# bxlab/bx-python

Measured on AMD Instinct MI355X. Metric: M overlap-queries/s at 100M x 10M intervals (count-only), higher is better.
Workload: dtype int32

## Files before the change

bx-python_amd/bxmi/_ffi.py:

```python
import ctypes as C
import os

import numpy as np

_HERE = os.path.dirname(os.path.abspath(__file__))
LIB_PATH = os.environ.get("BXMI_LIB") or os.path.join(_HERE, "libbxmi.so")

OK, EINVAL, ENOMEM, EHIP, ESTATE, ERANGE = 0, 1, 2, 3, 4, 5


class BxmiError(RuntimeError):
    def __init__(self, code, msg):
        super().__init__("libbxmi error %d: %s" % (code, msg))
        self.code = code


vp = C.c_void_p
i32, i64 = C.c_int32, C.c_int64
_p = C.POINTER

_SIGNATURES = {
    "bxmi_device_count": [_p(C.c_int)],
    "bxmi_set_device": [C.c_int],
    "bxmi_get_device": [_p(C.c_int)],
# ... 14 lines not shown
    "bxmi_ivl_append_dev": [vp, vp, vp, i64, vp],
    "bxmi_ivl_seal": [vp, vp],
    "bxmi_ivl_size": [vp, _p(i64)],
    "bxmi_ivl_has_reversed": [vp, _p(C.c_int)],
    "bxmi_ivl_order": [vp, vp],
    "bxmi_ivl_order_dev": [vp, _p(vp), _p(vp), _p(vp)],
    "bxmi_ivl_count": [vp, vp, vp, i64, vp, _p(i64)],
    "bxmi_ivl_count_dev": [vp, vp, vp, i64, vp, vp, vp],
    "bxmi_ivl_count_multi_dev": [vp, C.c_int, vp, vp, vp, vp, vp, vp],
    "bxmi_ivl_slice_state": [vp, _p(C.c_int), vp],
    "bxmi_ivl_dense_state": [vp, _p(C.c_int), vp],
    "bxmi_ivl_flat_state": [vp, _p(C.c_int), _p(i64)],
    "bxmi_ivl_sparse_state": [vp, _p(C.c_int), _p(i64), _p(C.c_int)],
    "bxmi_ivl_count_width": [vp, _p(C.c_int), _p(i64)],
    "bxmi_ivl_order_state": [vp, _p(C.c_int), _p(i64)],
    "bxmi_ivl_find": [vp, vp, vp, i64, vp, vp, i64, _p(i64)],
    "bxmi_ivl_find_dev": [vp, vp, vp, i64, vp, vp, i64, _p(i64), vp],
    "bxmi_ivl_find_one": [vp, i32, i32, vp, i64, _p(i64)],
    "bxmi_ivl_neighbors": [vp, i32, i32, C.c_int, vp, i64, _p(i64)],
    "bxmi_ivl_neighbors_batch": [vp, vp, i64, i32, i32, C.c_int, vp, vp, vp],
    "bxmi_ivl_neighbors_batch_dev": [vp, vp, i64, i32, i32, C.c_int, vp, vp, vp, vp],
    "bxmi_ivl_clusters": [vp, vp, i32, _p(i64), vp, vp, vp, vp],
    "bxmi_chainmap_create": [_p(vp), i64, vp, vp, vp, vp, vp, vp, vp, vp, vp],
    "bxmi_chainmap_destroy": [vp],
    "bxmi_chainmap_info": [vp, _p(i64), _p(i64), _p(i64)],
    "bxmi_chainmap_map": [vp, vp, vp, i64, i32, C.c_int, C.c_double, vp, vp, vp, vp, vp, i64, _p(i64)],
    "bxmi_chainmap_map_dev": [vp, vp, vp, i64, i32, C.c_int, C.c_double, vp, vp, vp, vp, vp, i64, _p(i64), vp],
    "bxmi_scores_create": [i64, _p(vp)],
    "bxmi_scores_destroy": [vp],
    "bxmi_scores_info": [vp, _p(i64)],
# ... 237 lines not shown
```

bx-python_amd/bxmi/intervals.py:

```python
import ctypes as C

import numpy as np

from . import _ffi
from ._ffi import as_i32, call, ptr


class IntervalIndex:

    def __init__(self):
        _ffi.require_gpu()
        h = C.c_void_p()
        call("bxmi_ivl_create", C.byref(h))
        self._h = h
        self._n = 0
        self._sealed = False
        self._one_buf = np.empty(4096, dtype=np.int32)

    def close(self):
        if getattr(self, "_h", None):
            _ffi.load().bxmi_ivl_destroy(self._h)
            self._h = None

    def __del__(self):
# ... 51 lines not shown
        st, hc, k = C.c_int(0), C.c_int64(0), C.c_int(0)
        call("bxmi_ivl_sparse_state", self._h, C.byref(st), C.byref(hc), C.byref(k))
        return st.value, hc.value, k.value

    def count_width(self):
        self._ready()
        bits, wide = C.c_int(0), C.c_int64(0)
        call("bxmi_ivl_count_width", self._h, C.byref(bits), C.byref(wide))
        return bits.value, wide.value

    def order_state(self):
        self._ready()
        sk, seen = C.c_int(0), C.c_int64(0)
        call("bxmi_ivl_order_state", self._h, C.byref(sk), C.byref(seen))
        return sk.value, seen.value

    def dense_state(self):
        self._ready()
        st, worst = C.c_int(0), (C.c_int64 * 2)()
        call("bxmi_ivl_dense_state", self._h, C.byref(st), worst)
        return st.value, list(worst)

    def order(self):
        self._ready()
        out = np.empty(self._n, dtype=np.int32)
        if self._n:
            call("bxmi_ivl_order", self._h, ptr(out))
        return out

    def count(self, qs, qe, want_counts=True):
# ... 129 lines not shown
```

bx-python_amd/csrc/count_dense.hpp:

```cpp
#pragma once
#include "offset_cells.hpp"

namespace bxmi {

constexpr int BD_UNIT_LOG2 = 19;
constexpr int BD_RSHIFT = 19;
constexpr int BD_MARGIN = 8192;
constexpr int BD_MAX_F = 6;
constexpr int BD_MAX_SHIFT = 19;
constexpr int BD_OV_MAX = 32704;
constexpr int BD_TABLE_FROM_FIRST = 2, BD_TABLE_FROM_LAST = 6;
constexpr int BD_THREADS = 1024;
constexpr int BD_LONG_SLOTS = 64;
constexpr int BD_LONG_CAP = 320;
constexpr int BD_HDR_QS = 6;

struct BdLayout {
    int nce, ncs;
    int bitsE, bitsS, metaE, metaS, hdr, ov, bytes;
    int ov_cap;
};

__host__ __device__ inline BdLayout bd_layout(int unit_log2)
{
// ... 1131 lines not shown
        for (int j = 0; j < 4; j++) b[j] = c[j] < 0xFFu ? c[j] : 0xFFu;
        reinterpret_cast<unsigned *>(out)[idx4] = b[0] | (b[1] << 8) | (b[2] << 16) | (b[3] << 24);
    } else {
        bd_v2u o;
        o.x = c[0] | (c[1] << 16), o.y = c[2] | (c[3] << 16);
        reinterpret_cast<bd_v2u *>(out)[idx4] = o;
    }
}

template <bool W8, int DEPTH, bool WIDE = false, int THREADS = BD_THREADS, bool TOT = false>
__global__ __launch_bounds__(THREADS) void bw_search_kernel(const BmSeg *__restrict__ segs, const int4 *__restrict__ items,
                                                               const int *__restrict__ n_items, const unsigned short *__restrict__ unitT, int64_t ntp,
                                                               const unsigned *__restrict__ recs ,
                                                               unsigned short *__restrict__ out , int tile_log2,
                                                               const unsigned *__restrict__ gate, unsigned *__restrict__ xcd_next ,
                                                               unsigned long long *__restrict__ total_slots = nullptr )
{
    if (gate && *gate == 0) return;
    extern __shared__ __attribute__((aligned(16))) int32_t dyn[];
    __shared__ long long s_red[TOT ? THREADS / 64 : 1];
    unsigned long long acc = 0ull;
    int acc_seg = -1;
    constexpr int LONG_CAP = THREADS == BD_THREADS ? BD_LONG_CAP : BD_LONG_CAP / 2;
    constexpr int PF = THREADS == BD_THREADS ? BW_PF : 10;
    __shared__ uint2 s_long[LONG_CAP];
    __shared__ int s_nlong, s_next, s_item_next;
    __shared__ __attribute__((aligned(8))) unsigned s_mask[THREADS / 64][BW_MASK_WORDS];
    const int nit = *n_items;
    const int per_xcd = (nit + 7) >> 3;
    const int xcd = (int)(blockIdx.x & 7);
    const int it_lo = xcd * per_xcd, it_hi = it_lo + per_xcd < nit ? it_lo + per_xcd : nit;
    const int lane = lane_id(), wave = __builtin_amdgcn_readfirstlane((int)(threadIdx.x >> 6));
    unsigned *const wmask = s_mask[wave];
    wmask[lane] = 0u, wmask[64 + lane] = 0u;
    if (threadIdx.x == 0) s_item_next = it_lo + (int)atomicAdd(&xcd_next[xcd], 1u);
    __syncthreads();
    int it = __builtin_amdgcn_readfirstlane(s_item_next);
    __syncthreads();
    const unsigned tile_slots = ((1u << tile_log2) + (unsigned)BM_PAD_ROOM) >> 2;
    while (it < it_hi) {
        const int4 item = items[it];
        const int unit = item.x & 0xffff, t0 = item.y, t1 = item.z;
        const BmSeg &sg = segs[item.x >> 16];
        if (TOT && (item.x >> 16) != acc_seg) {
            if (acc_seg >= 0) {
                block_accumulate_i64((long long)acc, s_red, total_slots + (int64_t)acc_seg * PT_SLOTS + (blockIdx.x & (PT_SLOTS - 1)));
                __syncthreads();
            }
            acc = 0ull, acc_seg = item.x >> 16;
        }
        const BmGeom g = sg.g;
        const int cell_log2 = WIDE ? 5 + g.dshift : 5;
        const BpLayout LP = bp_layout(g.shift + g.f, cell_log2, WIDE ? g.stride : 0);
        const unsigned short *__restrict__ runs0 = unitT + (int64_t)unit * ntp;
        const unsigned short *__restrict__ runs1 = runs0 + ntp;
        int B = BW_B;
// ... 397 lines not shown
                    } else {
#pragma unroll
                        for (int j = 0; j < 4; j++)
                            if (k0 + j >= lo && k0 + j < hi) as_global(sg.counts)[k0 + j] = (int)c[j];
                    }
                }
                acc += (long long)c[0] + c[1] + c[2] + c[3];
            }
        }
        __syncthreads();
        it = it_nx;
    }
    if (total_slots && acc_seg >= 0) block_accumulate_i64(acc, red, total_slots + (int64_t)acc_seg * PT_SLOTS + (blockIdx.x & (PT_SLOTS - 1)));
}

template <int THREADS, int ITEMS, bool PAD, bool W8>
__device__ __forceinline__ void bd_unpermute_tile(const unsigned short *__restrict__ cnt ,
                                                  const unsigned short *__restrict__ slots, const BmSeg *__restrict__ segs,
                                                  const unsigned short *__restrict__ tile_seg,
                                                  unsigned long long *__restrict__ total_slots ,
                                                  const unsigned *__restrict__ gate, const unsigned *__restrict__ tend,
                                                  unsigned long long *__restrict__ fb_dev ,
                                                  unsigned long long *__restrict__ fb_host )
{
    constexpr int TILE = THREADS * ITEMS;
    constexpr int STRIDE = PAD ? TILE + BM_PAD_ROOM : TILE;
    static_assert(ITEMS % 8 == 0, "whole 16-byte vectors of 16-bit counts per thread");
    extern __shared__ __attribute__((aligned(16))) int32_t dyn[];
    if (gate && *gate == 0) return;
    unsigned short *vals = reinterpret_cast<unsigned short *>(dyn);
    __shared__ long long red[THREADS / 64];
    const int64_t tile = blockIdx.x;
    const int seg_id = tile_seg[tile];
    const BmSeg &sg = segs[seg_id];
    const int64_t ltile = tile - sg.tile0;
    if (ltile >= sg.ntiles) return;
    unsigned long long *const acc_to = total_slots ? total_slots + (int64_t)seg_id * PT_SLOTS + (blockIdx.x & (PT_SLOTS - 1)) : nullptr;
    const IndexDev ix = sg.ix;
    const BmGeom g = sg.g;
    const int32_t *__restrict__ e_sorted = sg.e_sorted;
    const int32_t BX_GLOBAL *__restrict__ qs_arr = as_global(sg.qs) + ltile * TILE, *__restrict__ qe_arr = as_global(sg.qe) + ltile * TILE;
    int32_t BX_GLOBAL *__restrict__ out = as_global(sg.counts) + ltile * TILE;
    static_assert(!W8 || PAD, "8-bit counts come with the padded layout");
    const unsigned char *vals8 = reinterpret_cast<const unsigned char *>(dyn);
// ... 99 lines not shown
        if (__any(wide != 0u)) {
            unsigned w = wide;
#pragma unroll
            for (int off = 32; off > 0; off >>= 1) w += (unsigned)__shfl_down((int)w, off, 64);
            if (lane_id() == 0 && w) atomicAdd(fb_dev, (unsigned long long)w);
        }
        if (blockIdx.x == 0 && threadIdx.x == 0 && fb_host) *fb_host = __hip_atomic_load(fb_dev, __ATOMIC_RELAXED, __HIP_MEMORY_SCOPE_AGENT);
    }
}

template <int THREADS, int ITEMS, bool PAD = false, bool W8 = false>
__global__ __launch_bounds__(THREADS) void bd_unpermute_kernel(const unsigned short *__restrict__ cnt, const unsigned short *__restrict__ slots,
                                                               const BmSeg *__restrict__ segs, const unsigned short *__restrict__ tile_seg,
                                                               unsigned long long *__restrict__ total_slots, const unsigned *__restrict__ gate,
                                                               const unsigned *__restrict__ tend = nullptr, unsigned long long *__restrict__ fb_dev = nullptr,
                                                               unsigned long long *__restrict__ fb_host = nullptr)
{
    bd_unpermute_tile<THREADS, ITEMS, PAD, W8>(cnt, slots, segs, tile_seg, total_slots, gate, tend, fb_dev, fb_host);
}

}
```

bx-python_amd/csrc/count_plan.hpp:

```cpp
#pragma once
#include <cstddef>
#include <cstdint>
#include <vector>

namespace bxmi {

enum class Stage {
    None,
    Slices,
    Dense,
    Cells,
    OffsetCells,
};
constexpr int N_STAGES = 5;

constexpr int PLAN_NB = 2048;
constexpr int PLAN_GROUP_TILES = 64;
constexpr int PLAN_CHUNK = 65536;
constexpr int PLAN_PAR_CHUNK = 16;
constexpr int PLAN_PAD_ROOM = 4096 + 544;
constexpr int PLAN_PART_Q = 1024;
constexpr int PLAN_SLOTS = 64;
constexpr int PLAN_WALK_THREADS = 1024;
constexpr int PLAN_NBK = 2 * PLAN_NB;
constexpr int PLAN_BOUNDS_ROW = PLAN_NB + 2;
constexpr size_t PLAN_ITEM_BYTES = 16;

struct BmPlanKnobs {
    int64_t bm_variant = -1;
    int64_t sl_flat = 1;
    int64_t bd_chunk = 0;
    int64_t bm_chunk = 0;
    int64_t sl_lanes = 0;
    int64_t bd_w8 = -1;
    int64_t tot_walk = 1;
    int64_t sorted_path = 1;
    int64_t sorted_cells = 1;
    int64_t order_skip = -1;
};

struct BmPlanSegIn {
    int64_t nq = 0;
    int f = 0, shift = 0, stride = 0;
    bool want_counts = true, want_total = false;
    bool bd_blocks = false;
    int bo_state = 0;
    bool w8_off = false;
    int64_t n = 0, span = 1;
    size_t sl_lds = 0;
    int64_t sl_run = 0;
};

struct BmPlanIn {
    Stage stage = Stage::None;
    std::vector<BmPlanSegIn> seg;
    bool find = false, sub = false, direct = false;
    BmPlanKnobs knobs;
    size_t seg_bytes = 0;
    unsigned long long fb_wide_counts = 0;
    unsigned long long fb_order = 0;
    int64_t w8_queries = 0;
    unsigned long long order_seq = 0, order_seen = 0;
    int unsorted_streak = 0;
    bool order_skip = false;
};

enum class BmPlanError { None, TooManyQueries, TooManySegments, FindNeedsOneSliceIndex };

struct BmPlanSegOut {
    int64_t tile0, ntiles, tile_end;
};

struct BmPassPlan {
    BmPlanError error = BmPlanError::None;
    bool empty = false;
    int n = 0;
    int64_t nq_all = 0;
    bool wide = false, slices = false, cells = false, fxsub = false;
    bool slices_flat = false;
// ... 1 lines not shown
    int variant = 0;
    int tile_log2 = 14;
    bool pad = false;
    int64_t tile_stride = 0;
    std::vector<BmPlanSegOut> seg;
    int64_t ntp = 0;
    int ngroups = 0;
    int chunk = 0;
    int64_t max_items = 0;
    unsigned sgrid = 0;
    size_t search_lds = 0;
    bool big = false;
    bool any_blocks = false, any_total = false;
    int lanes = -1;
    bool tot_walk = false;
    bool w8_asked = false;
    bool w8 = false;
    bool w8_trip = false;
    bool multi_sorted = false;
    bool order_aware = false;
    bool sorted_on_cells = false;
    unsigned long long order_seen = 0;
    int unsorted_streak = 0;
    bool order_skip = false;
    bool probe_first = false;
    bool order_check = false;
    bool probe_rides = false;
    bool fold_params = false;
    unsigned sorted_chunk = 0;
    size_t sorted_items = 0;
// ... 8 lines not shown
    } bytes;
};

inline int64_t plan_div_up(int64_t a, int64_t b) { return (a + b - 1) / b; }

inline void bm_plan_set_order_skip(BmPassPlan &P, bool skip, const BmPlanKnobs &k)
{
    P.order_skip = skip;
    P.probe_rides = P.order_aware && skip && k.order_skip != 0;
    P.order_check = P.order_aware && !P.probe_rides;
    P.fold_params = P.n <= PLAN_PAR_CHUNK && !P.order_check;
    P.bytes.bs_plan = 0;
    if (P.order_check && (P.multi_sorted || P.sorted_on_cells)) P.bytes.bs_plan = P.bounds_bytes + (P.sorted_items + 1) * PLAN_ITEM_BYTES;
}

inline int bm_plan_variant(const BmPlanIn &in)
{
    const BmPlanKnobs &k = in.knobs;
    const int n = (int)in.seg.size();
    const bool wide = in.stage == Stage::OffsetCells, cells = in.stage == Stage::Cells || wide;
    int64_t nq_all = 0;
    for (const BmPlanSegIn &s : in.seg) nq_all += s.nq;
    int variant = k.bm_variant >= 0 ? (int)k.bm_variant : (nq_all >= ((int64_t)32 << 20) * (n == 1 ? 1 : 2) ? 2 : 0);
    if (cells && variant == 0 && k.bm_variant < 0) variant = 1;
    if (cells && variant == 0)
        for (const BmPlanSegIn &s : in.seg)
            if (s.f < 2) variant = 1;
    if (in.find && in.sub && variant == 0) variant = 1;
    return variant;
}
// ... 54 lines not shown
        for (int i = 0; i < n; i++) pad_slots += 3 * (int64_t)(PLAN_NB >> in.seg[(size_t)i].f) * (P.seg[(size_t)i].tile_end - P.seg[(size_t)i].tile0);
        max_items = 2 * ((nq_all + pad_slots) / chunk) + 2;
        for (int i = 0; i < n; i++) max_items += (PLAN_NB >> in.seg[(size_t)i].f) + 2;
    }
    P.max_items = max_items;
    P.sgrid = (unsigned)(plan_div_up(max_items, 8) * 8);

    bool pad = stage == Stage::Dense || cells;
    for (int i = 0; i < n && pad; i++) pad = (1 << in.seg[(size_t)i].f) >= (variant == 0 ? 4 : 2);
    P.pad = pad;
    const int64_t tile_stride = P.tile_stride = tile + (pad ? PLAN_PAD_ROOM : 0);

    bool tot_walk = k.tot_walk != 0 && cells && pad && !fx && P.any_total;
    for (int i = 0; i < n && tot_walk; i++) tot_walk = !in.seg[(size_t)i].want_counts;
    P.tot_walk = tot_walk;

    P.search_lds = slices ? sl_lds : max_stride * 16;
    if (slices_flat && P.search_lds < 4096) P.search_lds = 4096;
    P.big = wide && max_stride * 16 > (size_t)10 * (PLAN_WALK_THREADS / 2) * 16;
    if (slices && !slices_flat) {
        P.lanes = k.sl_lanes < 0 ? 0 : (k.sl_lanes ? (int)k.sl_lanes : (sl_run >= 96 ? 0 : (sl_run >= 40 ? 64 : 16)));
        if (fx && P.lanes == 0) P.lanes = 64;
    }

    if (pad && cells && k.bd_w8 != 0 && !tot_walk) {
        P.w8_asked = true;
        P.w8_trip = (int64_t)in.fb_wide_counts * 64 > in.w8_queries && in.fb_wide_counts > 4096;
        bool narrow = true;
        for (int i = 0; i < n; i++) {
            const BmPlanSegIn &s = in.seg[(size_t)i];
// ... 54 lines not shown
    }
    if (fxsub) {
        b.fx_tbl2 = T * PLAN_NBK * 2;
        b.fx_runT2 = T * PLAN_NBK * 4;
        b.fx_hc = T * (size_t)tile * 4;
        b.fx_svq = T * (size_t)tile * 4;
        b.fx_parts = T * (size_t)(tile / PLAN_PART_Q) * 8;
        b.fx_tile_tot = T * 8;
        b.fx_tile_base = (T + 2) * 8;
    }
    b.params = P.tile_off + T * sizeof(unsigned short);
    b.p_slots = ((size_t)n * PLAN_SLOTS + 8) * sizeof(unsigned long long);
    return P;
}

}
```

bx-python_amd/csrc/intervals.hip:

```cpp
#include <climits>
#include <vector>
#include <algorithm>
#include <atomic>
#include <condition_variable>
#include <mutex>
#include <thread>
#include <utility>

#include "primitives.hpp"
#include "count_plan.hpp"

#include "count_direct.hpp"
#include "count_parts.hpp"
#include "count_bitmap.hpp"
#include "count_slices.hpp"
#include "find_exchange.hpp"
#include "count_dense.hpp"
#include "find_sorted.hpp"
#include "find_direct.hpp"
#include "find_neighbors.hpp"
#include "cluster.hpp"

namespace bxmi {

// ... 16 lines not shown
static int64_t g_opt_sl_lanes = 0;
static int64_t g_opt_bm_hard_ppm = 2000;
static int64_t g_opt_flat = -1;
static int64_t g_opt_sparse = -1;
static int64_t g_opt_bo_cell_log2 = 0;
constexpr int64_t g_opt_bo_min_per_unit = 4096;
static int64_t g_opt_sorted_cells = 1;
static int64_t g_opt_dense = -1;
static int64_t g_opt_bd_chunk = 0;
static int64_t g_opt_bd_table_from = 0;
static int64_t g_opt_bd_blocks = 0;
static int64_t g_opt_bd_w8 = -1;
static int64_t g_opt_order_skip = -1;
static int64_t g_opt_clumped = -1;
static int64_t g_opt_tot_walk = 1;
static int64_t g_opt_host_chunk = 8 << 20;
static int64_t g_opt_host_touchers = 2;
constexpr int64_t g_opt_bd_unit_log2 = 0;

struct IvlOpt {
    const char *key;
    int64_t *var;
    int64_t (*norm)(int64_t);
};
static const IvlOpt IVL_OPTS[] = {
    {"ivl.partition", &g_opt_partition, nullptr},
    {"ivl.sorted_path", &g_opt_sorted_path, [](int64_t value) -> int64_t { return value != 0; }},
    {"ivl.bitmap_min", &g_opt_bitmap_min, nullptr},
    {"ivl.bitmap", &g_opt_bitmap, nullptr},
    {"ivl.bm_variant", &g_opt_bm_variant, [](int64_t value) -> int64_t { return value < 0 || value > 2 ? -1 : value; }},
// ... 5 lines not shown
    {"ivl.sl_flat", &g_opt_sl_flat, [](int64_t value) -> int64_t { return value != 0; }},
    {"ivl.sl_lanes", &g_opt_sl_lanes, [](int64_t value) -> int64_t { return value == 16 || value == 64 ? value : (value == 1 ? -1 : 0);  }},
    {"ivl.bm_hard_ppm", &g_opt_bm_hard_ppm, nullptr},
    {"ivl.flat", &g_opt_flat, nullptr},
    {"ivl.dense", &g_opt_dense, nullptr},
    {"ivl.sparse", &g_opt_sparse, nullptr},
    {"ivl.sorted_cells", &g_opt_sorted_cells, [](int64_t value) -> int64_t { return value != 0; }},
    {"ivl.bo_cell_log2", &g_opt_bo_cell_log2, [](int64_t value) -> int64_t { return value < BO_MIN_K || value > BO_MAX_K ? 0 : value; }},
    {"ivl.bd_chunk", &g_opt_bd_chunk, [](int64_t value) -> int64_t { return value < 0 ? 0 : value; }},
    {"ivl.bd_blocks", &g_opt_bd_blocks, [](int64_t value) -> int64_t { return value != 0; }},
    {"ivl.bd_table_from", &g_opt_bd_table_from, [](int64_t value) -> int64_t { return value < 1 || value > 64 ? 0 : value; }},
    {"ivl.bd_w8", &g_opt_bd_w8, nullptr},
    {"ivl.order_skip", &g_opt_order_skip, nullptr},
    {"ivl.clumped", &g_opt_clumped, nullptr},
    {"ivl.tot_walk", &g_opt_tot_walk, [](int64_t value) -> int64_t { return value != 0; }},
    {"ivl.host_chunk", &g_opt_host_chunk, [](int64_t value) -> int64_t { return value <= 0 ? 0 : ((value + 4095) & ~(int64_t)4095); }},
    {"ivl.host_touchers", &g_opt_host_touchers, [](int64_t value) -> int64_t { return value < 0 ? 0 : (value > 16 ? 16 : value); }},
};
constexpr int IVL_NOPTS = (int)(sizeof(IVL_OPTS) / sizeof(IVL_OPTS[0]));

int ivl_set_option(const char *key, int64_t value)
{
    for (int i = 0; i < IVL_NOPTS; i++)
        if (!strcmp(key, IVL_OPTS[i].key)) {
            *IVL_OPTS[i].var = IVL_OPTS[i].norm ? IVL_OPTS[i].norm(value) : value;
            return 1;
        }
    return 0;
}

// ... 49 lines not shown
    int bo_state = 0;
    bool bo_tried_clumped = false;
    int64_t bo_hard_cells = 0;
    BmGeom bo_geom{0, 0, 0, 0, 0, 0, 0, BP_RSHIFT, 0};
    DevBuf bo_images;
    DevBuf bs_plan;
    bool bd_blocks = false;
    DevBuf bd_images, bd_stats, bd_cnt16, bd_unitT, bd_tend;
    DevBuf bd_fb;
    unsigned long long *bd_fb_host = nullptr;
    int64_t w8_queries = 0;
    bool w8_off = false;
    unsigned long long order_seq = 0, order_seen = 0;
    int unsorted_streak = 0;
    bool order_skip = false;
    bool sl_eid_ready = false;
    int32_t *one_buf = nullptr;
    unsigned long long one_seq = 0;
    hipStream_t stream = nullptr;
    hipStream_t stream_up = nullptr, stream_down = nullptr;
    int device = 0;
};


static IndexDev index_dev(const bxmi_ivl *h);
template <typename Kern>
static int allow_big_lds(Kern k, size_t bytes)
{
    BXMI_HIP(hipFuncSetAttribute(reinterpret_cast<const void *>(k), hipFuncAttributeMaxDynamicSharedMemorySize, (int)bytes));
    return BXMI_OK;
// ... 378 lines not shown
    const BmSeg *segs;
    const unsigned short *tile_seg;
    bxmi_ivl *owner;
    int64_t ntp;
    int ngroups, tile_log2;
    size_t search_lds;
    const unsigned *gate;
    bool pad = false;
    bool w8 = false;
    bool wide = false;
    bool big = false;
    bool tot = false;
    unsigned long long *tot_slots = nullptr;
    unsigned *descent = nullptr;
    unsigned *xcd_next = nullptr;
    BmSegChunk par;
    int npar = 0;
    BmParOut par_out;
    int n_segs = 1;
    BmGeom g0;
    unsigned long long order_seq = 0;
};

template <int THREADS, int ITEMS>
static int bm_launch_tiles(const BmLaunch &L, hipStream_t st, bool sub = false)
{
    constexpr int TILE = THREADS * ITEMS;
    bxmi_ivl *h = L.owner;
    auto sort = [&](auto kern, int threads, size_t lds, unsigned *tend, unsigned short *tbl2, unsigned *tesc) {
        return launch_lds(kern, dim3((unsigned)L.ntp), dim3(threads), lds, st, L.segs, L.tile_seg, h->bm_recs.as<unsigned>(), h->bm_slots.as<unsigned short>(),
// ... 66 lines not shown
{
    bxmi_ivl *h = L.owner;
    return launch_lds(bd_search_kernel<FMT, QB, EXP, DEPTH, PIPE, PAD, W8>, dim3(grid), dim3(BD_THREADS), L.search_lds, st, L.segs, h->bm_items.as<int4>() + 1,
                      h->bm_items.as<int>(), h->bd_unitT.as<unsigned short>(), L.ntp, h->bm_recs.as<unsigned>(), h->bd_cnt16.as<unsigned short>(), L.tile_log2,
                      L.gate);
}

template <bool W8, bool WIDE, bool TOT = false, bool BIG = false>
static int bw_launch_search(const BmLaunch &L, hipStream_t st)
{
    bxmi_ivl *h = L.owner;
    constexpr int THREADS = WIDE && !BIG ? BD_THREADS / 2 : BD_THREADS;
    constexpr int DEPTH = 3;
    return launch_lds(bw_search_kernel<W8, DEPTH, WIDE, THREADS, TOT>, dim3(WIDE && !BIG ? 512 : 256), dim3(THREADS), L.search_lds, st, L.segs,
                      h->bm_items.as<int4>() + 1, h->bm_items.as<int>(), h->bd_unitT.as<unsigned short>(), L.ntp, h->bm_recs.as<unsigned>(),
                      h->bd_cnt16.as<unsigned short>(), L.tile_log2, L.gate, L.xcd_next, L.tot_slots);
}

static int bd_launch_search(const BmLaunch &L, unsigned grid, Stage fmt, bool blocks, hipStream_t st)
{
    if (fmt == Stage::Cells || fmt == Stage::OffsetCells) {
        if (!L.pad) return fail(BXMI_ESTATE, "bd_launch_search: cell images on packed runs");
        if (L.tot && L.big) return bw_launch_search<false, true, true, true>(L, st);
        if (L.tot) return L.wide ? bw_launch_search<false, true, true>(L, st) : bw_launch_search<false, false, true>(L, st);
        if (L.big) return L.w8 ? bw_launch_search<true, true, false, true>(L, st) : bw_launch_search<false, true, false, true>(L, st);
        if (L.wide) return L.w8 ? bw_launch_search<true, true>(L, st) : bw_launch_search<false, true>(L, st);
        return L.w8 ? bw_launch_search<true, false>(L, st) : bw_launch_search<false, false>(L, st);
    }
    if (fmt == Stage::Slices) return bd_launch_search_t<2, false, 0, 2, false>(L, grid, st);
#ifndef BD_EXP_V
#define BD_EXP_V 0
#endif
    if (L.pad) return blocks ? bd_launch_search_t<0, true, BD_EXP_V, 3, true, true>(L, grid, st) : bd_launch_search_t<0, false, BD_EXP_V, 3, true, true>(L, grid, st);
    return blocks ? bd_launch_search_t<0, true, BD_EXP_V, 4, true>(L, grid, st) : bd_launch_search_t<0, false, BD_EXP_V, 4, true>(L, grid, st);
}

template <int THREADS, int ITEMS>
static int bd_launch_unpermute(const BmLaunch &L, unsigned long long *slots, hipStream_t st)
{
    bxmi_ivl *h = L.owner;
    const bool w8 = L.pad && L.w8;
    auto unpermute = [&](auto kern, size_t count_bytes) {
        return launch_lds(kern, dim3((unsigned)L.ntp), dim3(THREADS), (size_t)(THREADS * ITEMS + (L.pad ? BM_PAD_ROOM : 0)) * count_bytes, st,
                          h->bd_cnt16.as<unsigned short>(), h->bm_slots.as<unsigned short>(), L.segs, L.tile_seg, slots, L.gate,
                          L.pad ? h->bd_tend.as<unsigned>() : nullptr, w8 ? h->bd_fb.as<unsigned long long>() : nullptr, w8 ? h->bd_fb_host : nullptr);
    };
    if (w8) return unpermute(bd_unpermute_kernel<THREADS, ITEMS, true, true>, 1);
    if (L.pad) return unpermute(bd_unpermute_kernel<THREADS, ITEMS, true>, sizeof(unsigned short));
    return unpermute(bd_unpermute_kernel<THREADS, ITEMS, false>, sizeof(unsigned short));
}

static int bs_launch_walk(const BmLaunch &L, const int4 *items, const int *n_items, unsigned long long *tslots, hipStream_t st)
{
    auto walk = [&](auto kern, unsigned grid, unsigned threads) {
        return launch_lds(kern, dim3(grid), dim3(threads), L.search_lds, st, L.segs, items, n_items, tslots, L.gate, L.xcd_next, L.owner->bd_fb_host + 1, L.order_seq);
    };
    if (L.wide && L.big) return walk(bs_walk_kernel<true, BD_THREADS>, 256, BD_THREADS);
    if (L.wide) return walk(bs_walk_kernel<true, BD_THREADS / 2>, 512, BD_THREADS / 2);
    return walk(bs_walk_kernel<false, BD_THREADS>, 256, BD_THREADS);
}
// ... 19 lines not shown
    BXMI_TRY(h->bd_fb.reserve(64));
    BXMI_HIP(hipMemsetAsync(h->bd_fb.p, 0, 64, st));
    return BXMI_OK;
}

static_assert(PLAN_NB == BM_NB && PLAN_GROUP_TILES == BM_GROUP_TILES && PLAN_CHUNK == BM_CHUNK && PLAN_PAR_CHUNK == BM_PAR_CHUNK &&
                  PLAN_PAD_ROOM == BM_PAD_ROOM && PLAN_PART_Q == BM_PART_Q && PLAN_SLOTS == PT_SLOTS && PLAN_WALK_THREADS == BD_THREADS &&
                  PLAN_NBK == FX_NBK && PLAN_BOUNDS_ROW == BS_BOUNDS_ROW && PLAN_ITEM_BYTES == sizeof(int4),
              "count_plan.hpp and the device headers disagree on a layout constant");

static BmPlanKnobs bm_plan_knobs()
{
    BmPlanKnobs k;
    k.bm_variant = g_opt_bm_variant, k.sl_flat = g_opt_sl_flat, k.bd_chunk = g_opt_bd_chunk, k.bm_chunk = g_opt_bm_chunk, k.sl_lanes = g_opt_sl_lanes;
    k.bd_w8 = g_opt_bd_w8, k.tot_walk = g_opt_tot_walk, k.sorted_path = g_opt_sorted_path, k.sorted_cells = g_opt_sorted_cells;
    k.order_skip = g_opt_order_skip;
    return k;
}

static int bm_reserve(bxmi_ivl *h, const BmPassPlan::Bytes &b)
{
    const struct { DevBuf *buf; size_t bytes; } want[] = {
        {&h->bm_tesc, b.tesc}, {&h->bm_recs, b.recs}, {&h->bd_tend, b.tend}, {&h->bm_slots, b.slots}, {&h->bm_tbl, b.tbl}, {&h->bm_runT, b.runT},
        {&h->bd_unitT, b.unitT}, {&h->bm_grpcnt, b.grpcnt}, {&h->sl_unitcnt, b.unitcnt}, {&h->bd_cnt16, b.cnt16}, {&h->bm_items, b.items},
        {&h->sl_cnt, b.sl_cnt}, {&h->sl_loff, b.sl_loff}, {&h->fx_tbl2, b.fx_tbl2}, {&h->fx_runT2, b.fx_runT2}, {&h->fx_hc, b.fx_hc}, {&h->fx_svq, b.fx_svq},
        {&h->fx_parts, b.fx_parts}, {&h->fx_tile_tot, b.fx_tile_tot}, {&h->fx_tile_base, b.fx_tile_base}, {&h->bm_params, b.params}, {&h->p_slots, b.p_slots}};
    for (const auto &w : want) BXMI_TRY(w.buf->reserve(w.bytes));
    return BXMI_OK;
}

static int bm_set_params(BmLaunch &L, const BmPassPlan &P, const std::vector<BmSeg> &segs, int64_t *const *totals_dev, unsigned long long *slots, hipStream_t st)
// ... 91 lines not shown
        sg.nq = nq[i];
        sg.dimages = hs[i]->bd_images.as<unsigned char>();
        sg.pimages = wide ? hs[i]->bo_images.as<unsigned char>() : hs[i]->bp_images.as<unsigned char>();
        sg.smeta = slices ? hs[i]->sl_meta.as<int4>() : nullptr;
        sg.ix = index_dev(hs[i]);
        sg.e_sorted = hs[i]->e_sorted.as<int32_t>();
        si.f = sg.g.f, si.shift = sg.g.shift, si.stride = sg.g.stride;
        si.want_counts = counts[i] != nullptr, si.want_total = totals_dev && totals_dev[i];
        si.bd_blocks = hs[i]->bd_blocks, si.bo_state = hs[i]->bo_state, si.w8_off = hs[i]->w8_off;
        si.n = hs[i]->n, si.span = (int64_t)hs[i]->cmax - (int64_t)hs[i]->geom.cmin + 1;
    }
    const volatile unsigned long long *fb = h->bd_fb_host;
    in.fb_wide_counts = fb ? fb[0] : 0, in.fb_order = fb ? fb[1] : 0;
    in.w8_queries = h->w8_queries;
    in.order_seq = h->order_seq, in.order_seen = h->order_seen, in.unsorted_streak = h->unsorted_streak, in.order_skip = h->order_skip;

    BmPassPlan P = bm_plan_pass(in);
    if (P.error == BmPlanError::TooManyQueries) return fail(BXMI_EINVAL, "bxmi_ivl_count: more than 2^31 queries in one batch");
    if (P.error == BmPlanError::TooManySegments) return fail(BXMI_EINVAL, "bxmi_ivl_count_multi: more than 4096 indexes in one batch");
    if (P.error != BmPlanError::None) return fail(BXMI_ESTATE, "bm_count_segments: the half-bucket order serves find() on one index's slices");
    if (P.empty) return BXMI_OK;
    for (int i = 0; i < n; i++) segs[(size_t)i].tile0 = P.seg[(size_t)i].tile0, segs[(size_t)i].ntiles = P.seg[(size_t)i].ntiles, segs[(size_t)i].tile_end = P.seg[(size_t)i].tile_end;

    BXMI_TRY(bm_reserve(h, P.bytes));
    if (P.fxsub) fx->f = segs[0].g.f, fx->ntiles = segs[0].ntiles;
    unsigned long long *slots = h->p_slots.as<unsigned long long>();
    unsigned *order_word = reinterpret_cast<unsigned *>(slots + (size_t)n * PT_SLOTS);

    if (P.order_aware || P.w8_asked) BXMI_TRY(ensure_feedback(h, st));
    BmLaunch L;
    if (P.order_aware) {
        h->order_seen = P.order_seen, h->unsorted_streak = P.unsorted_streak, h->order_skip = P.order_skip;
        if (P.probe_first) {
            hipLaunchKernelGGL(bm_probe_kernel, dim3(1), dim3(256), 0, st, qs[0], nq[0], order_word);
            unsigned seen_descent = 0;
            BXMI_HIP(hipMemcpyAsync(&seen_descent, order_word, sizeof(unsigned), hipMemcpyDeviceToHost, st));
            BXMI_HIP(hipStreamSynchronize(st));
            if (seen_descent) {
                h->unsorted_streak = 2, h->order_skip = true;
                bm_plan_set_order_skip(P, true, in.knobs);
            }
        }
        L.order_seq = ++h->order_seq;
    }
    BXMI_TRY(h->bs_plan.reserve(P.bytes.bs_plan));
// ... 27 lines not shown
    if (P.fxsub) {
        hipLaunchKernelGGL(bm_transpose_kernel<FX_NBK>, dim3((unsigned)P.ngroups, FX_NBK / 64), dim3(256), 0, st, h->fx_tbl2.as<unsigned short>(), L.segs,
                           L.tile_seg, P.tile_log2, h->fx_runT2.as<unsigned>(), P.ntp, (unsigned *)nullptr, L.gate);
        BXMI_LAUNCH_CHECK();
    }
    if (P.dense) {
        hipLaunchKernelGGL(bd_transpose_kernel, dim3((unsigned)P.ngroups, BM_NB / 64), dim3(256), 0, st, h->bm_tbl.as<unsigned short>(), L.segs, L.tile_seg,
                           P.tile_log2, h->bd_unitT.as<unsigned short>(), P.ntp, h->sl_unitcnt.as<unsigned>(), L.gate,
                           P.pad ? h->bd_tend.as<unsigned>() : (const unsigned *)nullptr);
    } else {
        hipLaunchKernelGGL(bm_transpose_kernel<BM_NB>, dim3((unsigned)P.ngroups, BM_NB / 64), dim3(256), 0, st, h->bm_tbl.as<unsigned short>(), L.segs, L.tile_seg,
                           P.tile_log2, h->bm_runT.as<unsigned>(), P.ntp, h->bm_grpcnt.as<unsigned>(), L.gate);
        hipLaunchKernelGGL(sl_unit_sums_kernel, dim3((unsigned)P.ngroups), dim3(1024), 0, st, h->bm_grpcnt.as<unsigned>(), L.segs, L.tile_seg,
                           h->sl_unitcnt.as<unsigned>(), L.gate);
    }
    BXMI_TRY(bm_launch_plan(L, P.chunk, st));
    unsigned *search_out = fx ? h->sl_cnt.as<unsigned>() : h->bm_recs.as<unsigned>();
    if (P.slices_flat)
        BXMI_TRY(bd_launch_search(L, P.sgrid, Stage::Slices, false, st));
    else if (slices) {
        if (P.lanes == 0)
            BXMI_TRY(sl_launch_search_flat(L, P.sgrid, st));
        else if (P.lanes == 64)
            BXMI_TRY(sl_launch_search<64>(L, P.sgrid, st, search_out, P.fxsub ? h->fx_hc.as<unsigned>() : nullptr));
        else
            BXMI_TRY(sl_launch_search<16>(L, P.sgrid, st, search_out, P.fxsub ? h->fx_hc.as<unsigned>() : nullptr));
        if (fx) fx->L = L, fx->sgrid = P.sgrid, fx->lanes = P.lanes, fx->variant = P.variant;
    } else
        BXMI_TRY(bd_launch_search(L, P.sgrid, stage, P.any_blocks, st));
    unsigned *loff = fx ? h->sl_loff.as<unsigned>() : nullptr;
    if (P.tot_walk) {
// ... 342 lines not shown
        h->geom.cmin = cmin;
        h->geom.shift = shift;
        h->cmax = cmax;
        h->sl_state = 0;
        for (unsigned &need : h->sl_need) need = 0;
        h->fx_state = 0, h->fx_pieces_f = -1, h->fx_hits_per_q = -1.0;
        h->bd_state = 0, h->bd_worst[0] = h->bd_worst[1] = 0, h->bd_blocks = false;
        h->bp_state = 0, h->bp_hard_cells = 0;
        h->bo_state = 0, h->bo_tried_clumped = false, h->bo_hard_cells = 0;
        h->w8_off = false, h->w8_queries = 0;
        if (h->bd_fb_host) {
            BXMI_HIP(hipMemsetAsync(h->bd_fb.p, 0, 64, st));
            *h->bd_fb_host = 0;
        }
        h->unsorted_streak = 0, h->order_skip = false;
        h->sl_eid_ready = false;
        BXMI_TRY(h->slice_bounds.reserve(PT_NB * sizeof(SliceBound)));
        hipLaunchKernelGGL(part_bounds_kernel, dim3(PT_NB / 256), dim3(256), 0, st, h->s_ord.as<int32_t>(), h->e_sorted.as<int32_t>(),
                           h->pm.as<int32_t>(), (int)n, h->geom, h->slice_bounds.as<SliceBound>());
        BXMI_LAUNCH_CHECK();
        h->images_ready = false;
        BXMI_HIP(hipStreamSynchronize(st));
    }
    h->sealed = true;
    return BXMI_OK;
}

extern "C" int bxmi_ivl_size(const bxmi_ivl_t *h, int64_t *n)
{
    if (!h || !n) return fail(BXMI_EINVAL, "bxmi_ivl_size: bad arguments");
// ... 36 lines not shown
extern "C" int bxmi_ivl_count_width(const bxmi_ivl_t *h, int *bits, int64_t *wide_counts)
{
    BXMI_TRY(need_sealed(h, "bxmi_ivl_count_width"));
    const unsigned long long wide = h->bd_fb_host ? *reinterpret_cast<volatile unsigned long long *>(h->bd_fb_host) : 0ull;
    const int64_t span = (int64_t)h->cmax - (int64_t)h->geom.cmin + 1;
    if (bits) *bits = !h->w8_off && (int64_t)h->n * 2048 < span * 128 ? 8 : 16;
    if (wide_counts) *wide_counts = (int64_t)wide;
    return BXMI_OK;
}

extern "C" int bxmi_ivl_order_state(const bxmi_ivl_t *h, int *skipping, int64_t *answers_seen)
{
    BXMI_TRY(need_sealed(h, "bxmi_ivl_order_state"));
    if (skipping) *skipping = h->order_skip && g_opt_order_skip != 0 ? 1 : 0;
    if (answers_seen) *answers_seen = (int64_t)h->order_seen;
    return BXMI_OK;
}

extern "C" int bxmi_ivl_dense_state(const bxmi_ivl_t *h, int *state, int64_t *worst)
{
    BXMI_TRY(need_sealed(h, "bxmi_ivl_dense_state"));
    if (state) *state = h->bd_state;
    if (worst) worst[0] = h->bd_worst[0], worst[1] = h->bd_worst[1];
    return BXMI_OK;
}

extern "C" int bxmi_ivl_slice_state(const bxmi_ivl_t *h, int *state, int64_t *unit_keys)
{
    BXMI_TRY(need_sealed(h, "bxmi_ivl_slice_state"));
    if (state) *state = h->sl_state;
// ... 521 lines not shown
```

include/bxmi.h:

```cpp
#ifndef BXMI_H
#define BXMI_H

#include <stddef.h>
#include <stdint.h>

#ifdef __cplusplus
extern "C" {
#endif

#define BXMI_OK 0
#define BXMI_EINVAL 1
#define BXMI_ENOMEM 2
#define BXMI_EHIP 3
#define BXMI_ESTATE 4
#define BXMI_ERANGE 5

typedef struct bxmi_ivl bxmi_ivl_t;
typedef struct bxmi_bits bxmi_bits_t;

int bxmi_version(void);
const char *bxmi_last_error(void);
int bxmi_device_count(int *n);
int bxmi_set_device(int device);
int bxmi_get_device(int *device);
// ... 20 lines not shown
int bxmi_ivl_has_reversed(const bxmi_ivl_t *h, int *flag);
int bxmi_ivl_order(const bxmi_ivl_t *h, int32_t *idx_out);
int bxmi_ivl_order_dev(const bxmi_ivl_t *h, const int32_t **idx_dev, const int32_t **start_dev, const int32_t **end_dev);

int bxmi_ivl_count(bxmi_ivl_t *h, const int32_t *qs, const int32_t *qe, int64_t nq, int32_t *counts, int64_t *total);
int bxmi_ivl_count_dev(bxmi_ivl_t *h, const int32_t *qs, const int32_t *qe, int64_t nq, int32_t *counts,
                       int64_t *total_dev, void *stream);
int bxmi_ivl_count_multi_dev(bxmi_ivl_t *const *hs, int n, const int32_t *const *qs, const int32_t *const *qe, const int64_t *nq,
                             int32_t *const *counts, int64_t *const *totals_dev, void *stream);
int bxmi_ivl_slice_state(const bxmi_ivl_t *h, int *state, int64_t *unit_keys);
int bxmi_ivl_dense_state(const bxmi_ivl_t *h, int *state, int64_t *worst);
int bxmi_ivl_flat_state(const bxmi_ivl_t *h, int *state, int64_t *hard_cells);
int bxmi_ivl_sparse_state(const bxmi_ivl_t *h, int *state, int64_t *hard_cells, int *cell_log2);
int bxmi_ivl_count_width(const bxmi_ivl_t *h, int *bits, int64_t *wide_counts);
int bxmi_ivl_order_state(const bxmi_ivl_t *h, int *skipping, int64_t *answers_seen);

int bxmi_ivl_find(bxmi_ivl_t *h, const int32_t *qs, const int32_t *qe, int64_t nq, int64_t *offsets,
                  int32_t *hits, int64_t cap, int64_t *total);
int bxmi_ivl_find_dev(bxmi_ivl_t *h, const int32_t *qs, const int32_t *qe, int64_t nq, int64_t *offsets,
                      int32_t *hits, int64_t cap, int64_t *total_host, void *stream);

int bxmi_ivl_find_one(bxmi_ivl_t *h, int32_t qs, int32_t qe, int32_t *hits, int64_t cap, int64_t *n_hits);

int bxmi_ivl_neighbors(bxmi_ivl_t *h, int32_t position, int32_t max_dist, int dir, int32_t *out, int64_t cap,
                       int64_t *n_out);

int bxmi_ivl_neighbors_batch(bxmi_ivl_t *h, const int32_t *pos, int64_t nq, int32_t k, int32_t max_dist, int dir, int32_t *out,
                             int32_t *n_out, int64_t *n_cand);
int bxmi_ivl_neighbors_batch_dev(bxmi_ivl_t *h, const int32_t *pos, int64_t nq, int32_t k, int32_t max_dist, int dir, int32_t *out,
                                 int32_t *n_out, int64_t *n_cand, void *stream);
// ... 199 lines not shown
```

Baseline: 150,600.

## Skip the plan kernel using device feedback on unit balance, with a static item schedule

Adds a feedback path in which the unpermute kernel reports the largest per-unit query count back to the host. When earlier batches showed balanced units and a similar tile count, the count pass skips the planning launch. The search kernel then derives its work items statically from the segment, with a tail of possibly-empty units checked on device and skipped. This removes a kernel launch and its item-building work per batch, at the cost of heuristic state, one-batch-lagged feedback and more complex indexing in the search loop.

```diff
diff --git a/bx-python_amd/bxmi/_ffi.py b/bx-python_amd/bxmi/_ffi.py
--- a/bx-python_amd/bxmi/_ffi.py
+++ b/bx-python_amd/bxmi/_ffi.py
@@ -52,6 +52,7 @@
     "bxmi_ivl_sparse_state": [vp, _p(C.c_int), _p(i64), _p(C.c_int)],
     "bxmi_ivl_count_width": [vp, _p(C.c_int), _p(i64)],
     "bxmi_ivl_order_state": [vp, _p(C.c_int), _p(i64)],
+    "bxmi_ivl_plan_state": [vp, _p(C.c_int), _p(i64), _p(i64)],
     "bxmi_ivl_find": [vp, vp, vp, i64, vp, vp, i64, _p(i64)],
     "bxmi_ivl_find_dev": [vp, vp, vp, i64, vp, vp, i64, _p(i64), vp],
     "bxmi_ivl_find_one": [vp, i32, i32, vp, i64, _p(i64)],
diff --git a/bx-python_amd/bxmi/intervals.py b/bx-python_amd/bxmi/intervals.py
--- a/bx-python_amd/bxmi/intervals.py
+++ b/bx-python_amd/bxmi/intervals.py
@@ -89,6 +89,12 @@
         sk, seen = C.c_int(0), C.c_int64(0)
         call("bxmi_ivl_order_state", self._h, C.byref(sk), C.byref(seen))
         return sk.value, seen.value
+
+    def plan_state(self):
+        self._ready()
+        st, seen, largest = C.c_int(0), C.c_int64(0), C.c_int64(0)
+        call("bxmi_ivl_plan_state", self._h, C.byref(st), C.byref(seen), C.byref(largest))
+        return st.value, seen.value, largest.value
 
     def dense_state(self):
         self._ready()
diff --git a/bx-python_amd/csrc/count_dense.hpp b/bx-python_amd/csrc/count_dense.hpp
--- a/bx-python_amd/csrc/count_dense.hpp
+++ b/bx-python_amd/csrc/count_dense.hpp
@@ -1169,7 +1169,10 @@
                                                                const unsigned *__restrict__ recs ,
                                                                unsigned short *__restrict__ out , int tile_log2,
                                                                const unsigned *__restrict__ gate, unsigned *__restrict__ xcd_next ,
-                                                               unsigned long long *__restrict__ total_slots = nullptr )
+                                                               unsigned long long *__restrict__ total_slots = nullptr ,
+                                                               int static_units = 0 ,
+                                                               const unsigned *__restrict__ unitcnt = nullptr ,
+                                                               int ngroups = 0)
 {
     if (gate && *gate == 0) return;
     extern __shared__ __attribute__((aligned(16))) int32_t dyn[];
@@ -1181,10 +1184,14 @@
     __shared__ uint2 s_long[LONG_CAP];
     __shared__ int s_nlong, s_next, s_item_next;
     __shared__ __attribute__((aligned(8))) unsigned s_mask[THREADS / 64][BW_MASK_WORDS];
-    const int nit = *n_items;
+    const bool planned = TOT || static_units == 0;
+    const int nit = planned ? *n_items : static_units;
     const int per_xcd = (nit + 7) >> 3;
     const int xcd = (int)(blockIdx.x & 7);
-    const int it_lo = xcd * per_xcd, it_hi = it_lo + per_xcd < nit ? it_lo + per_xcd : nit;
+    const int it_lo = xcd * per_xcd;
+    const int static_tail = planned ? 0 : (BM_NB >> segs[0].g.f) - static_units;
+    const int tail_x = static_tail > xcd ? (static_tail - xcd + 7) >> 3 : 0;
+    const int it_hi = (it_lo + per_xcd < nit ? it_lo + per_xcd : (it_lo < nit ? nit : it_lo)) + tail_x;
     const int lane = lane_id(), wave = __builtin_amdgcn_readfirstlane((int)(threadIdx.x >> 6));
     unsigned *const wmask = s_mask[wave];
     wmask[lane] = 0u, wmask[64 + lane] = 0u;
@@ -1194,7 +1201,27 @@
     __syncthreads();
     const unsigned tile_slots = ((1u << tile_log2) + (unsigned)BM_PAD_ROOM) >> 2;
     while (it < it_hi) {
-        const int4 item = items[it];
+        int4 item;
+        if (planned) {
+            item = items[it];
+        } else {
+            const BmSeg &s0g = segs[0];
+            const int64_t per_unit = s0g.nq / static_units;
+            const bool behind = it - it_lo < tail_x;
+            item = make_int4(behind ? static_units + xcd + 8 * (it - it_lo) : it - tail_x, (int)s0g.tile0, (int)(s0g.tile0 + s0g.ntiles),
+                             (int)(per_unit < 0x7fffffff ? per_unit : 0x7fffffff));
+            if (behind) {
+                unsigned any = 0u;
+                for (int gi = threadIdx.x; gi < ngroups; gi += THREADS) any |= unitcnt[(int64_t)gi * BM_NB + item.x];
+                if (!__syncthreads_or(any != 0u)) {
+                    if (threadIdx.x == 0) s_item_next = it_lo + (int)atomicAdd(&xcd_next[xcd], 1u);
+                    __syncthreads();
+                    it = __builtin_amdgcn_readfirstlane(s_item_next);
+                    __syncthreads();
+                    continue;
+                }
+            }
+        }
         const int unit = item.x & 0xffff, t0 = item.y, t1 = item.z;
         const BmSeg &sg = segs[item.x >> 16];
         if (TOT && (item.x >> 16) != acc_seg) {
@@ -1622,6 +1649,42 @@
     if (total_slots && acc_seg >= 0) block_accumulate_i64(acc, red, total_slots + (int64_t)acc_seg * PT_SLOTS + (blockIdx.x & (PT_SLOTS - 1)));
 }
 
+struct BdUnitsFb {
+    const unsigned *unitcnt;
+    int ngroups;
+    unsigned seq;
+    unsigned long long *dev;
+    unsigned long long *host;
+};
+
+template <int THREADS>
+__device__ __forceinline__ void bd_report_units(const BdUnitsFb &uf)
+{
+    __shared__ unsigned s_largest;
+    if (threadIdx.x == 0) s_largest = 0u;
+    __syncthreads();
+    unsigned largest = 0u;
+    for (int u = threadIdx.x; u < BM_NB; u += THREADS) {
+        unsigned sum = 0u;
+        for (int g = 0; g < uf.ngroups; g++) sum += uf.unitcnt[(int64_t)g * BM_NB + u];
+        largest = sum > largest ? sum : largest;
+    }
+#pragma unroll
+    for (int off = 32; off > 0; off >>= 1) {
+        const unsigned o = (unsigned)__shfl_down((int)largest, off, 64);
+        largest = o > largest ? o : largest;
+    }
+    if (lane_id() == 0) atomicMax(&s_largest, largest);
+    __syncthreads();
+    if (threadIdx.x == 0) {
+        const unsigned long long before = *uf.dev;
+        const unsigned mine = s_largest < 0xFFFFFFFEu ? s_largest : 0xFFFFFFFEu;
+        const unsigned prev = uf.seq > 1u && (unsigned)(before >> 32) + 1u == uf.seq ? (unsigned)before : 0xFFFFFFFFu;
+        *uf.dev = ((unsigned long long)uf.seq << 32) | mine;
+        *uf.host = ((unsigned long long)uf.seq << 32) | (prev > mine ? prev : mine);
+    }
+}
+
 template <int THREADS, int ITEMS, bool PAD, bool W8>
 __device__ __forceinline__ void bd_unpermute_tile(const unsigned short *__restrict__ cnt ,
                                                   const unsigned short *__restrict__ slots, const BmSeg *__restrict__ segs,
@@ -1629,13 +1692,14 @@
                                                   unsigned long long *__restrict__ total_slots ,
                                                   const unsigned *__restrict__ gate, const unsigned *__restrict__ tend,
                                                   unsigned long long *__restrict__ fb_dev ,
-                                                  unsigned long long *__restrict__ fb_host )
+                                                  unsigned long long *__restrict__ fb_host , const BdUnitsFb &uf)
 {
     constexpr int TILE = THREADS * ITEMS;
     constexpr int STRIDE = PAD ? TILE + BM_PAD_ROOM : TILE;
     static_assert(ITEMS % 8 == 0, "whole 16-byte vectors of 16-bit counts per thread");
     extern __shared__ __attribute__((aligned(16))) int32_t dyn[];
     if (gate && *gate == 0) return;
+    if (PAD && uf.host && blockIdx.x == 0) bd_report_units<THREADS>(uf);
     unsigned short *vals = reinterpret_cast<unsigned short *>(dyn);
     __shared__ long long red[THREADS / 64];
     const int64_t tile = blockIdx.x;
@@ -1765,9 +1829,10 @@
                                                                const BmSeg *__restrict__ segs, const unsigned short *__restrict__ tile_seg,
                                                                unsigned long long *__restrict__ total_slots, const unsigned *__restrict__ gate,
                                                                const unsigned *__restrict__ tend = nullptr, unsigned long long *__restrict__ fb_dev = nullptr,
-                                                               unsigned long long *__restrict__ fb_host = nullptr)
-{
-    bd_unpermute_tile<THREADS, ITEMS, PAD, W8>(cnt, slots, segs, tile_seg, total_slots, gate, tend, fb_dev, fb_host);
-}
-
-}
+                                                               unsigned long long *__restrict__ fb_host = nullptr,
+                                                               BdUnitsFb uf = BdUnitsFb{nullptr, 0, 0u, nullptr, nullptr})
+{
+    bd_unpermute_tile<THREADS, ITEMS, PAD, W8>(cnt, slots, segs, tile_seg, total_slots, gate, tend, fb_dev, fb_host, uf);
+}
+
+}
diff --git a/bx-python_amd/csrc/count_plan.hpp b/bx-python_amd/csrc/count_plan.hpp
--- a/bx-python_amd/csrc/count_plan.hpp
+++ b/bx-python_amd/csrc/count_plan.hpp
@@ -37,6 +37,7 @@
     int64_t sorted_path = 1;
     int64_t sorted_cells = 1;
     int64_t order_skip = -1;
+    int64_t static_plan = 1;
 };
 
 struct BmPlanSegIn {
@@ -63,6 +64,12 @@
     unsigned long long order_seq = 0, order_seen = 0;
     int unsorted_streak = 0;
     bool order_skip = false;
+    unsigned long long fb_units = 0;
+    unsigned long long units_seen = 0;
+    bool units_balanced = false;
+    int64_t units_tiles_lo = 0, units_tiles_hi = 0;
+    int64_t fb_units_tiles[2] = {0, 0};
+    int64_t span_units = 0;
 };
 
 enum class BmPlanError { None, TooManyQueries, TooManySegments, FindNeedsOneSliceIndex };
@@ -94,6 +101,13 @@
     bool any_blocks = false, any_total = false;
     int lanes = -1;
     bool tot_walk = false;
+    bool units_fb = false;
+    unsigned long long units_seen = 0;
+    bool units_balanced = false;
+    int64_t units_tiles_lo = 0, units_tiles_hi = 0;
+    bool static_plan = false;
+    int static_units = 0;
+    int static_tail = 0;
     bool w8_asked = false;
     bool w8 = false;
     bool w8_trip = false;
@@ -132,6 +146,9 @@
     if (P.order_check && (P.multi_sorted || P.sorted_on_cells)) P.bytes.bs_plan = P.bounds_bytes + (P.sorted_items + 1) * PLAN_ITEM_BYTES;
 }
 
+constexpr int64_t PLAN_STATIC_TILES_TOL = 2;
+inline void bm_plan_static(BmPassPlan &P, const BmPlanIn &in, int chunk);
+
 inline int bm_plan_variant(const BmPlanIn &in)
 {
     const BmPlanKnobs &k = in.knobs;
@@ -216,6 +233,8 @@
     bool tot_walk = k.tot_walk != 0 && cells && pad && !fx && P.any_total;
     for (int i = 0; i < n && tot_walk; i++) tot_walk = !in.seg[(size_t)i].want_counts;
     P.tot_walk = tot_walk;
+
+    bm_plan_static(P, in, chunk);
 
     P.search_lds = slices ? sl_lds : max_stride * 16;
     if (slices_flat && P.search_lds < 4096) P.search_lds = 4096;
@@ -300,4 +319,27 @@
     return P;
 }
 
-}
+inline void bm_plan_static(BmPassPlan &P, const BmPlanIn &in, int chunk)
+{
+    P.units_seen = in.units_seen, P.units_balanced = in.units_balanced;
+    P.units_tiles_lo = in.units_tiles_lo, P.units_tiles_hi = in.units_tiles_hi;
+    P.units_fb = in.knobs.static_plan != 0 && P.n == 1 && P.cells && P.pad && !in.find && !P.tot_walk;
+    if (!P.units_fb) return;
+    if ((in.fb_units >> 32) > in.units_seen) {
+        const unsigned long long largest = in.fb_units & 0xFFFFFFFFull;
+        const int64_t a = in.fb_units_tiles[0], b = in.fb_units_tiles[1];
+        P.units_seen = in.fb_units >> 32;
+        P.units_balanced = largest != 0xFFFFFFFFull && largest <= (unsigned long long)chunk && a > 0 && b > 0;
+        P.units_tiles_lo = a < b ? a : b, P.units_tiles_hi = a < b ? b : a;
+    }
+    const int64_t tiles = P.seg[0].ntiles;
+    P.static_plan = P.units_balanced && in.span_units > 0 && tiles <= PLAN_STATIC_TILES_TOL * P.units_tiles_lo &&
+                    tiles * PLAN_STATIC_TILES_TOL >= P.units_tiles_hi;
+    if (P.static_plan) {
+        const int all = PLAN_NB >> in.seg[0].f;
+        P.static_units = (int)(in.span_units < all ? in.span_units : all);
+        P.static_tail = all - P.static_units;
+    }
+}
+
+}
diff --git a/bx-python_amd/csrc/intervals.hip b/bx-python_amd/csrc/intervals.hip
--- a/bx-python_amd/csrc/intervals.hip
+++ b/bx-python_amd/csrc/intervals.hip
@@ -54,6 +54,7 @@
 static int64_t g_opt_order_skip = -1;
 static int64_t g_opt_clumped = -1;
 static int64_t g_opt_tot_walk = 1;
+static int64_t g_opt_static_plan = 1;
 static int64_t g_opt_host_chunk = 8 << 20;
 static int64_t g_opt_host_touchers = 2;
 constexpr int64_t g_opt_bd_unit_log2 = 0;
@@ -89,6 +90,7 @@
     {"ivl.order_skip", &g_opt_order_skip, nullptr},
     {"ivl.clumped", &g_opt_clumped, nullptr},
     {"ivl.tot_walk", &g_opt_tot_walk, [](int64_t value) -> int64_t { return value != 0; }},
+    {"ivl.static_plan", &g_opt_static_plan, [](int64_t value) -> int64_t { return value != 0; }},
     {"ivl.host_chunk", &g_opt_host_chunk, [](int64_t value) -> int64_t { return value <= 0 ? 0 : ((value + 4095) & ~(int64_t)4095); }},
     {"ivl.host_touchers", &g_opt_host_touchers, [](int64_t value) -> int64_t { return value < 0 ? 0 : (value > 16 ? 16 : value); }},
 };
@@ -168,6 +170,11 @@
     unsigned long long order_seq = 0, order_seen = 0;
     int unsorted_streak = 0;
     bool order_skip = false;
+    unsigned long long units_seq = 0, units_seen = 0;
+    bool units_balanced = false;
+    int64_t units_tiles_lo = 0, units_tiles_hi = 0;
+    int64_t units_tiles[64] = {0};
+    bool static_plan = false;
     bool sl_eid_ready = false;
     int32_t *one_buf = nullptr;
     unsigned long long one_seq = 0;
@@ -576,6 +583,8 @@
     unsigned long long *tot_slots = nullptr;
     unsigned *descent = nullptr;
     unsigned *xcd_next = nullptr;
+    int static_units = 0;
+    BdUnitsFb units_fb{nullptr, 0, 0u, nullptr, nullptr};
     BmSegChunk par;
     int npar = 0;
     BmParOut par_out;
@@ -672,7 +681,7 @@
     constexpr int DEPTH = 3;
     return launch_lds(bw_search_kernel<W8, DEPTH, WIDE, THREADS, TOT>, dim3(WIDE && !BIG ? 512 : 256), dim3(THREADS), L.search_lds, st, L.segs,
                       h->bm_items.as<int4>() + 1, h->bm_items.as<int>(), h->bd_unitT.as<unsigned short>(), L.ntp, h->bm_recs.as<unsigned>(),
-                      h->bd_cnt16.as<unsigned short>(), L.tile_log2, L.gate, L.xcd_next, L.tot_slots);
+                      h->bd_cnt16.as<unsigned short>(), L.tile_log2, L.gate, L.xcd_next, L.tot_slots, L.static_units, L.units_fb.unitcnt, L.units_fb.ngroups);
 }
 
 static int bd_launch_search(const BmLaunch &L, unsigned grid, Stage fmt, bool blocks, hipStream_t st)
@@ -701,7 +710,8 @@
     auto unpermute = [&](auto kern, size_t count_bytes) {
         return launch_lds(kern, dim3((unsigned)L.ntp), dim3(THREADS), (size_t)(THREADS * ITEMS + (L.pad ? BM_PAD_ROOM : 0)) * count_bytes, st,
                           h->bd_cnt16.as<unsigned short>(), h->bm_slots.as<unsigned short>(), L.segs, L.tile_seg, slots, L.gate,
-                          L.pad ? h->bd_tend.as<unsigned>() : nullptr, w8 ? h->bd_fb.as<unsigned long long>() : nullptr, w8 ? h->bd_fb_host : nullptr);
+                          L.pad ? h->bd_tend.as<unsigned>() : nullptr, w8 ? h->bd_fb.as<unsigned long long>() : nullptr, w8 ? h->bd_fb_host : nullptr,
+                          L.units_fb);
     };
     if (w8) return unpermute(bd_unpermute_kernel<THREADS, ITEMS, true, true>, 1);
     if (L.pad) return unpermute(bd_unpermute_kernel<THREADS, ITEMS, true>, sizeof(unsigned short));
@@ -751,7 +761,7 @@
     BmPlanKnobs k;
     k.bm_variant = g_opt_bm_variant, k.sl_flat = g_opt_sl_flat, k.bd_chunk = g_opt_bd_chunk, k.bm_chunk = g_opt_bm_chunk, k.sl_lanes = g_opt_sl_lanes;
     k.bd_w8 = g_opt_bd_w8, k.tot_walk = g_opt_tot_walk, k.sorted_path = g_opt_sorted_path, k.sorted_cells = g_opt_sorted_cells;
-    k.order_skip = g_opt_order_skip;
+    k.order_skip = g_opt_order_skip, k.static_plan = g_opt_static_plan;
     return k;
 }
 
@@ -873,6 +883,14 @@
     in.fb_wide_counts = fb ? fb[0] : 0, in.fb_order = fb ? fb[1] : 0;
     in.w8_queries = h->w8_queries;
     in.order_seq = h->order_seq, in.order_seen = h->order_seen, in.unsorted_streak = h->unsorted_streak, in.order_skip = h->order_skip;
+    in.fb_units = fb ? fb[2] : 0;
+    in.units_seen = h->units_seen, in.units_balanced = h->units_balanced, in.units_tiles_lo = h->units_tiles_lo, in.units_tiles_hi = h->units_tiles_hi;
+    {
+        const unsigned long long s = in.fb_units >> 32;
+        const bool known = s >= 2 && s <= h->units_seq && h->units_seq - s < 63;
+        in.fb_units_tiles[0] = known ? h->units_tiles[s & 63] : 0, in.fb_units_tiles[1] = known ? h->units_tiles[(s - 1) & 63] : 0;
+    }
+    in.span_units = (((int64_t)h->cmax - (int64_t)segs[0].g.cmin) >> (segs[0].g.shift + segs[0].g.f)) + 1;
 
     BmPassPlan P = bm_plan_pass(in);
     if (P.error == BmPlanError::TooManyQueries) return fail(BXMI_EINVAL, "bxmi_ivl_count: more than 2^31 queries in one batch");
@@ -886,8 +904,16 @@
     unsigned long long *slots = h->p_slots.as<unsigned long long>();
     unsigned *order_word = reinterpret_cast<unsigned *>(slots + (size_t)n * PT_SLOTS);
 
-    if (P.order_aware || P.w8_asked) BXMI_TRY(ensure_feedback(h, st));
+    if (P.order_aware || P.w8_asked || P.units_fb) BXMI_TRY(ensure_feedback(h, st));
     BmLaunch L;
+    h->static_plan = P.static_plan;
+    if (P.units_fb) {
+        h->units_seen = P.units_seen, h->units_balanced = P.units_balanced, h->units_tiles_lo = P.units_tiles_lo, h->units_tiles_hi = P.units_tiles_hi;
+        ++h->units_seq;
+        h->units_tiles[h->units_seq & 63] = P.seg[0].ntiles;
+        L.units_fb = BdUnitsFb{h->sl_unitcnt.as<unsigned>(), P.ngroups, (unsigned)h->units_seq, h->bd_fb.as<unsigned long long>() + 2, h->bd_fb_host + 2};
+        L.static_units = P.static_plan ? P.static_units : 0;
+    }
     if (P.order_aware) {
         h->order_seen = P.order_seen, h->unsorted_streak = P.unsorted_streak, h->order_skip = P.order_skip;
         if (P.probe_first) {
@@ -945,7 +971,7 @@
         hipLaunchKernelGGL(sl_unit_sums_kernel, dim3((unsigned)P.ngroups), dim3(1024), 0, st, h->bm_grpcnt.as<unsigned>(), L.segs, L.tile_seg,
                            h->sl_unitcnt.as<unsigned>(), L.gate);
     }
-    BXMI_TRY(bm_launch_plan(L, P.chunk, st));
+    if (!P.static_plan) BXMI_TRY(bm_launch_plan(L, P.chunk, st));
     unsigned *search_out = fx ? h->sl_cnt.as<unsigned>() : h->bm_recs.as<unsigned>();
     if (P.slices_flat)
         BXMI_TRY(bd_launch_search(L, P.sgrid, Stage::Slices, false, st));
@@ -1318,6 +1344,7 @@
             *h->bd_fb_host = 0;
         }
         h->unsorted_streak = 0, h->order_skip = false;
+        h->units_seen = h->units_seq, h->units_balanced = false, h->static_plan = false;
         h->sl_eid_ready = false;
         BXMI_TRY(h->slice_bounds.reserve(PT_NB * sizeof(SliceBound)));
         hipLaunchKernelGGL(part_bounds_kernel, dim3(PT_NB / 256), dim3(256), 0, st, h->s_ord.as<int32_t>(), h->e_sorted.as<int32_t>(),
@@ -1384,6 +1411,16 @@
     BXMI_TRY(need_sealed(h, "bxmi_ivl_order_state"));
     if (skipping) *skipping = h->order_skip && g_opt_order_skip != 0 ? 1 : 0;
     if (answers_seen) *answers_seen = (int64_t)h->order_seen;
+    return BXMI_OK;
+}
+
+extern "C" int bxmi_ivl_plan_state(const bxmi_ivl_t *h, int *static_plan, int64_t *answers_seen, int64_t *largest_unit)
+{
+    BXMI_TRY(need_sealed(h, "bxmi_ivl_plan_state"));
+    const unsigned long long word = h->bd_fb_host ? reinterpret_cast<volatile unsigned long long *>(h->bd_fb_host)[2] : 0ull;
+    if (static_plan) *static_plan = h->static_plan ? 1 : 0;
+    if (answers_seen) *answers_seen = (int64_t)h->units_seen;
+    if (largest_unit) *largest_unit = (word & 0xFFFFFFFFull) == 0xFFFFFFFFull ? -1 : (int64_t)(word & 0xFFFFFFFFull);
     return BXMI_OK;
 }
 
diff --git a/include/bxmi.h b/include/bxmi.h
--- a/include/bxmi.h
+++ b/include/bxmi.h
@@ -58,6 +58,7 @@
 int bxmi_ivl_sparse_state(const bxmi_ivl_t *h, int *state, int64_t *hard_cells, int *cell_log2);
 int bxmi_ivl_count_width(const bxmi_ivl_t *h, int *bits, int64_t *wide_counts);
 int bxmi_ivl_order_state(const bxmi_ivl_t *h, int *skipping, int64_t *answers_seen);
+int bxmi_ivl_plan_state(const bxmi_ivl_t *h, int *static_plan, int64_t *answers_seen, int64_t *largest_unit);
 
 int bxmi_ivl_find(bxmi_ivl_t *h, const int32_t *qs, const int32_t *qe, int64_t nq, int64_t *offsets,
                   int32_t *hits, int64_t cap, int64_t *total);
```

Result: faster. 152,200 (median of 6 runs) (+1.1%).
